# pmh47/dirt

Measured on AMD Instinct MI355X. Metric: forward+backward Mpixels/s at 1024x1024x4ch, 10k-tri mesh, higher is better.
Workload: dtype f32 (f64 edge functions); 1 GPU; K3: rand_mesh F=10000 at 1024x1024x4, 1 scene(s) per GPU, forward+backward; scenes_per_gpu=1, parallelism=batch-sharded x1, no collective, launch=eager (Python wrapper + C ABI per step)

## Files before the change

### dirt_amd/csrc/dirt_forward.hip

```cpp
#include <type_traits>
#include "dirt_device.h"
#include "dirt_launch.h"
#include "dirt_raster_common.h"
#include "../../include/dirt_hip.h"

namespace dirt {

#ifdef DIRT_TRACE
__device__ long long* g_trace_fwd_setup = nullptr;
__device__ long long* g_trace_fwd_raster = nullptr;
extern "C" void dirt_debug_set_trace_forward(void* ps, void* pr)
{
    long long* q = reinterpret_cast<long long*>(ps);
    (void)hipMemcpyToSymbol(HIP_SYMBOL(g_trace_fwd_setup), &q, sizeof(q));
    q = reinterpret_cast<long long*>(pr);
    (void)hipMemcpyToSymbol(HIP_SYMBOL(g_trace_fwd_raster), &q, sizeof(q));
}
#define FMARK() do { if (tr_n < 12) { long long t_; asm volatile("s_memtime %0\n\ts_waitcnt lgkmcnt(0)" : "=s"(t_) :: "memory"); tr_t[tr_n++] = t_; } } while (0)
#define FTRACE_DECL() long long tr_t[12]; int tr_n = 0; const long long tr_wall0 = wall_clock64()
#else
#define FMARK() do {} while (0)
#define FTRACE_DECL() do {} while (0)
#endif

namespace {

constexpr int MAX_FACE_BINS = 16;

__device__ __forceinline__ void glds16(const void* base, uint32_t voff, uint32_t lds_addr)
{
    unsigned keep;
    asm volatile("s_mov_b32 %0, m0\n\ts_mov_b32 m0, %3\n\ts_nop 0\n\tglobal_load_lds_dwordx4 %1, %2\n\ts_mov_b32 m0, %0"
                 : "=&s"(keep) : "v"(voff), "s"(base), "s"(lds_addr) : "memory");
}

#define DIRT_LDS __attribute__((address_space(3)))

constexpr int WAIT_VMCNT_0 = 0x0F70;

template <class T>
__device__ __forceinline__ uint32_t lds_address(T* p)
{
    return (uint32_t)(uintptr_t)(__attribute__((address_space(3))) void*)p;
}

}

constexpr int STHREADS = 256;
template <int CK>
__global__ __launch_bounds__(STHREADS) void setup_kernel_v2(const float* __restrict__ a_vertices, const int32_t* __restrict__ a_faces,
                                                            const float* __restrict__ a_vertex_colors, int a_shared_faces, int a_V, int a_F,
                                                            GeomParams g_in)
{
    GeomParams g = g_in;
    g.vertices = a_vertices; g.faces = a_faces; g.vertex_colors = a_vertex_colors; g.shared_faces = a_shared_faces; g.V = a_V; g.F = a_F;
    __shared__ __align__(16) unsigned long long s_mask[MAX_BINS_MASKED + 2];
    __shared__ __align__(16) FaceRec s_recs[64];
    __shared__ __align__(16) TileRec s_lrecs[64];
    __shared__ __align__(16) float4 s_crecs[CK ? 3 * 64 : 1];
    __shared__ FaceBox s_box[64];
    __shared__ uint8_t s_ok_edges[64], s_ok_box[64];
    const int ib = blockIdx.y, chunk = blockIdx.x, tid = threadIdx.x, lane = tid & 63;
    const int role = __builtin_amdgcn_readfirstlane(tid >> 6);
    FTRACE_DECL();
    FMARK();
    const int nbins = g.grid.bins_x * g.grid.bins_y, big = g.grid.big;
    BinCell* __restrict__ row = g.cells + ((size_t)ib * g.nchunk + chunk) * (size_t)g.grid.cell_chunk_stride;
    if (g.F == 0 || g.V <= 0) {
        for (int i = tid; i <= big; i += STHREADS) if (i < nbins || i == big) row[i] = BinCell{0u, 0u};
        return;
    }
    const int f0 = chunk * 64;
    const int nf = min(64, g.F - f0);
    const size_t n0 = (size_t)ib * g.F + f0;
    const int f = f0 + lane;
    const bool have = lane < nf;
    const int fs = have ? f : 0;
    const float* __restrict__ verts = g.vertices + (size_t)ib * g.V * 4;
    const float* __restrict__ cols = CK ? g.vertex_colors + (size_t)ib * g.V * CK : nullptr;
    auto fetch = [&](int vid) {
        if (role != 3) return *reinterpret_cast<const float4*>(verts + (size_t)vid * 4);
        if constexpr (CK == 0) return make_float4(0.f, 0.f, 0.f, 0.f);
        else {
            const float* __restrict__ cp = cols + (size_t)vid * CK;
            if constexpr (CK == 4) return *reinterpret_cast<const float4*>(cp);
            else if constexpr (CK == 3) { const Float3 q = *reinterpret_cast<const Float3*>(cp); return make_float4(q.x, q.y, q.z, 0.f); }
            else return make_float4(cp[0], 0.f, 0.f, 0.f);
        }
    };
    int32_t idx[3] = {0, 0, 0};
    float4 vv[3];
    const bool fetches = role != 2 && (role != 3 || CK != 0);
    if (fetches) {
        const int32_t* __restrict__ fp = g.faces + (g.shared_faces ? (size_t)fs : (size_t)ib * g.F + fs) * 3;
        idx[0] = fp[0]; idx[1] = fp[1]; idx[2] = fp[2];
#pragma unroll
        for (int k = 0; k < 3; ++k) vv[k] = fetch(min(3 * fs + k, g.V - 1));
    } else if (role == 2) {
        for (int i = lane; i < nbins; i += 64) s_mask[i] = 0ull;
        if (lane == 0) s_mask[big] = 0ull;
    }
    FMARK();
    if (fetches) {
        const bool identity = 3 * fs + 2 < g.V && idx[0] == 3 * fs && idx[1] == 3 * fs + 1 && idx[2] == 3 * fs + 2;
        if (__builtin_amdgcn_ballot_w64(have && !identity) != 0ull) {
#pragma unroll
            for (int k = 0; k < 3; ++k) {
                const int ci = identity ? 3 * fs + k : ((uint32_t)idx[k] < (uint32_t)g.V ? idx[k] : 0);
                vv[k] = fetch(ci);
            }
        }
    }
    FMARK();
    bool ok_mine = false;
    FaceBox box;
    box.i_min = 0; box.i_max = -1; box.r_min = 0; box.r_max = -1;
    if (role == 0) {
        FaceRec rec;
        ok_mine = have && setup_face_edges(vv, idx, g.V, g.H, g.W, rec);
        if (ok_mine) s_recs[lane] = rec;
        else s_recs[lane].flags = 0;
        s_ok_edges[lane] = ok_mine ? 1 : 0;
    } else if (role == 1) {
        ok_mine = have && setup_face_box(vv, g.H, g.W, box);
        s_box[lane] = box;
        s_ok_box[lane] = ok_mine ? 1 : 0;
    } else if (role == 3) {
        if constexpr (CK != 0) { s_crecs[3 * lane] = vv[0]; s_crecs[3 * lane + 1] = vv[1]; s_crecs[3 * lane + 2] = vv[2]; }
    }
    FMARK();
    __syncthreads();
    if (role == 1) {
        if (ok_mine && s_ok_edges[lane]) {
            const unsigned long long bit = 1ull << lane;
            const int bx0 = box.i_min >> g.grid.shift, bx1 = box.i_max >> g.grid.shift;
            const int by0 = box.r_min >> g.grid.shift, by1 = box.r_max >> g.grid.shift;
            if ((bx1 - bx0 + 1) * (by1 - by0 + 1) <= MAX_FACE_BINS) {
                for (int by = by0; by <= by1; ++by)
                    for (int bx = bx0; bx <= bx1; ++bx) atomicOr(&s_mask[by * g.grid.bins_x + bx], bit);
            } else {
                atomicOr(&s_mask[big], bit);
            }
            if (!g.v2_only) {
                BinEntry e;
                e.box = box; e.face = f; e.pad = 0;
                g.entries[((size_t)ib * g.nchunk + chunk) * (5 * (size_t)g.chunk_faces) + lane] = e;
            }
        }
    } else if (role == 2) {
        if (have && s_ok_edges[lane] && s_ok_box[lane]) {
            TileRec lr;
            make_local_rec(s_recs[lane], f, s_box[lane], g.H, (float)g.W, (float)g.H, &lr);
            s_lrecs[lane] = lr;
        }
    } else if (role == 0) {
        const uint4* __restrict__ src = reinterpret_cast<const uint4*>(&s_recs[0]);
        uint4* __restrict__ dst = reinterpret_cast<uint4*>(g.recs + n0);
        for (int i = lane; i < 8 * nf; i += 64) dst[i] = src[i];
    } else {
        if constexpr (CK != 0) {
            const uint4* __restrict__ src = reinterpret_cast<const uint4*>(&s_crecs[0]);
            uint4* __restrict__ dst = reinterpret_cast<uint4*>(g.crecs + 3 * n0);
            for (int i = lane; i < 3 * nf; i += 64) dst[i] = src[i];
        }
    }
    __syncthreads();
    FMARK();
    {
        const uint4* __restrict__ src = reinterpret_cast<const uint4*>(&s_lrecs[0]);
        uint4* __restrict__ dst = reinterpret_cast<uint4*>(g.lrecs + n0);
        for (int i = tid; i < 5 * nf; i += STHREADS) dst[i] = src[i];
    }
    for (int i = 2 * tid; i < nbins; i += 2 * STHREADS) {
        if (i + 1 < nbins) {
            const ulonglong2 m = *reinterpret_cast<const ulonglong2*>(&s_mask[i]);
            *reinterpret_cast<ulonglong2*>(&row[i]) = m;
        } else {
            const unsigned long long m = s_mask[i];
            row[i] = BinCell{(uint32_t)m, (uint32_t)(m >> 32)};
        }
    }
    if (tid == STHREADS - 1) {
        const unsigned long long m = s_mask[big];
        row[big] = BinCell{(uint32_t)m, (uint32_t)(m >> 32)};
    }
    FMARK();
#ifdef DIRT_TRACE
    if (tid == 0 && g_trace_fwd_setup) {
        long long* o = g_trace_fwd_setup + ((size_t)blockIdx.y * gridDim.x + blockIdx.x) * 16;
        for (int i = 0; i < 12; ++i) o[i] = i < tr_n ? tr_t[i] : 0;
        o[12] = tr_wall0; o[13] = (long long)wall_clock64() - tr_wall0;
    }
#endif
}

hipError_t launch_geometry_v2(const GeomParams& g, hipStream_t stream)
{
    const dim3 grid((unsigned)g.nchunk, (unsigned)g.B);
    const int ck = g.crecs ? g.C : 0;
    if (ck == 4) hipLaunchKernelGGL(setup_kernel_v2<4>, grid, dim3(STHREADS), 0, stream, g.vertices, g.faces, g.vertex_colors, g.shared_faces, g.V, g.F, g);
    else if (ck == 3) hipLaunchKernelGGL(setup_kernel_v2<3>, grid, dim3(STHREADS), 0, stream, g.vertices, g.faces, g.vertex_colors, g.shared_faces, g.V, g.F, g);
    else if (ck == 1) hipLaunchKernelGGL(setup_kernel_v2<1>, grid, dim3(STHREADS), 0, stream, g.vertices, g.faces, g.vertex_colors, g.shared_faces, g.V, g.F, g);
    else hipLaunchKernelGGL(setup_kernel_v2<0>, grid, dim3(STHREADS), 0, stream, g.vertices, g.faces, g.vertex_colors, g.shared_faces, g.V, g.F, g);
    return hipGetLastError();
}

namespace {

#ifndef DIRT_V2_CAP
#define DIRT_V2_CAP 96
#endif
constexpr int V2_CAP = DIRT_V2_CAP;

template <bool COLOURS>
struct alignas(16) ShadeSlot {
    double coef[9];
    double inv_det;
    uint32_t flags;
    int32_t vid[3];
    float4 col[COLOURS ? 3 : 0];
};
static_assert(sizeof(ShadeSlot<true>) == 144 && sizeof(ShadeSlot<false>) == 96, "16-byte pieces: 6 of the record, 3 colours");

}

#ifndef DIRT_V2_WAVES
#define DIRT_V2_WAVES 6
#endif
template <int MODE, int CSPEC, int WAVES = 4>
__global__ __launch_bounds__(64 * WAVES, WAVES == 8 ? 8 : DIRT_V2_WAVES) void raster_kernel_v2(
    const BinCell* __restrict__ a_cells, int a_nchunk, int a_tiles_x, int a_tiles_y, uint32_t a_tiles_x_magic, int a_shift, int a_bins_x,
    int a_big, int a_chunk_stride, RasterParams p_in)
{
    RasterParams p = p_in;
    p.cells = a_cells; p.nchunk = a_nchunk; p.tiles_x = a_tiles_x; p.tiles_y = a_tiles_y; p.tiles_x_magic = a_tiles_x_magic;
    p.grid.shift = a_shift; p.grid.bins_x = a_bins_x; p.grid.big = a_big; p.grid.cell_chunk_stride = a_chunk_stride;
    constexpr int NB = 2, NBY = WAVES == 8 ? 1 : 2, TILE = 32, PPL = NB * NBY, THREADS = 64 * WAVES, RH = 8 * NBY;
    constexpr bool COLOURS = MODE == 0;
    constexpr int SPARTS = COLOURS ? 9 : 6;
    using Slot = ShadeSlot<COLOURS>;
    __shared__ __align__(16) TileRec s_rec[V2_CAP];
    __shared__ __align__(16) Slot s_shade[V2_CAP];
    __shared__ int32_t s_face[V2_CAP];
    __shared__ uint32_t s_count;
    FTRACE_DECL();
    FMARK();
#ifdef DIRT_TRACE
    int tr_cand = 0;
#endif
    const int tid = threadIdx.x;
    const int lane = tid & 63;
    const int wave = __builtin_amdgcn_readfirstlane(tid >> 6);
    const int ib = blockIdx.y;
    const int tile = xcd_tile(blockIdx.x, p.tiles_x * p.tiles_y);
    int tile_col, tile_row;
    tile_xy(tile, p.tiles_x, p.tiles_x_magic, tile_col, tile_row);
    const int tx0 = tile_col * TILE, tr0 = tile_row * TILE;
    constexpr int C = CSPEC;

    const FaceRec* __restrict__ recs = p.recs + (size_t)ib * p.F;
    const TileRec* __restrict__ lrecs = p.lrecs + (size_t)ib * p.F;
    const float4* __restrict__ crecs = COLOURS ? p.crecs + (size_t)ib * p.F * 3 : nullptr;
    const int bin = (tr0 >> p.grid.shift) * p.grid.bins_x + (tx0 >> p.grid.shift);
    const BinCell* __restrict__ cells = p.cells + (size_t)ib * p.nchunk * (size_t)p.grid.cell_chunk_stride;
    unsigned long long m_bin = 0ull, m_big = 0ull;
    if (tid < p.nchunk) {
        const BinCell* __restrict__ rowc = cells + (size_t)tid * p.grid.cell_chunk_stride;
        const BinCell a = rowc[bin], b = rowc[p.grid.big];
        m_bin = ((unsigned long long)a.count << 32) | a.start;
        m_big = ((unsigned long long)b.count << 32) | b.start;
    }

    const int wx = wave & 1, wy = wave >> 1;
    const int x0 = tx0 + wx * 16 + (lane & 7);
    const int r0 = tr0 + wy * RH + (lane >> 3);
    double px[NB], py[NBY];
#pragma unroll
    for (int k = 0; k < NB; ++k) px[k] = (double)(x0 + 8 * k) + 0.5;
#pragma unroll
    for (int k = 0; k < NBY; ++k) py[k] = (double)(p.H - 1 - (r0 + 8 * k)) + 0.5;
    unsigned long long best[PPL];
    int cbest[PPL];
#pragma unroll
    for (int k = 0; k < PPL; ++k) { best[k] = (unsigned long long)Z24_CLEAR << 32; cbest[k] = V2_CAP; }
    bool lds_records = true;

    const uint32_t lds_rec = (uint32_t)__builtin_amdgcn_readfirstlane((int)lds_address(&s_rec[0]));
    const uint32_t lds_shade = (uint32_t)__builtin_amdgcn_readfirstlane((int)lds_address(&s_shade[0]));

    FMARK();
    for (int round = 0;; ++round) {
        if (tid == 0) s_count = 0;
        __syncthreads();
        FMARK();
        if (64 * wave < p.nchunk) {
            const uint32_t cnt = (uint32_t)__popcll(m_bin) + (uint32_t)__popcll(m_big);
            uint32_t incl = cnt;
            incl += (uint32_t)__builtin_amdgcn_update_dpp(0, (int)incl, 0x111 , 0xF, 0xF, false);
            incl += (uint32_t)__builtin_amdgcn_update_dpp(0, (int)incl, 0x112 , 0xF, 0xF, false);
            incl += (uint32_t)__builtin_amdgcn_update_dpp(0, (int)incl, 0x114 , 0xF, 0xF, false);
            incl += (uint32_t)__builtin_amdgcn_update_dpp(0, (int)incl, 0x118 , 0xF, 0xF, false);
            incl += (uint32_t)__builtin_amdgcn_update_dpp(0, (int)incl, 0x142 , 0xA, 0xF, false);
            incl += (uint32_t)__builtin_amdgcn_update_dpp(0, (int)incl, 0x143 , 0xC, 0xF, false);
            const uint32_t total = (uint32_t)__builtin_amdgcn_readlane((int)incl, 63);
            uint32_t base = 0;
            if (total != 0u) {
                if (lane == 0) base = atomicAdd(&s_count, total);
                base = (uint32_t)__builtin_amdgcn_readfirstlane((int)base);
            }
            uint32_t slot = base + incl - cnt;
            const int face0 = tid * 64;
            while (m_bin != 0ull && slot < (uint32_t)V2_CAP) {
                s_face[slot++] = face0 + (__ffsll((long long)m_bin) - 1);
                m_bin &= m_bin - 1ull;
            }
            while (m_big != 0ull && slot < (uint32_t)V2_CAP) {
                s_face[slot++] = face0 + (__ffsll((long long)m_big) - 1);
                m_big &= m_big - 1ull;
            }
        }
        FMARK();
        __syncthreads();
        FMARK();
        const int n = (int)min(s_count, (uint32_t)V2_CAP);
        if (round != 0) lds_records = false;

        int tid_o = tid;
        asm volatile("" : "+v"(tid_o));
#pragma unroll
        for (int k = 0; k < (5 * V2_CAP + THREADS - 1) / THREADS; ++k) {
            const int idx = tid_o + THREADS * k;
            if (idx < 5 * n) {
                const int slot = idx / 5, part = idx - 5 * slot;
                glds16(lrecs, (uint32_t)s_face[slot] * (uint32_t)sizeof(TileRec) + 16u * (uint32_t)part, lds_rec + 1024u * (uint32_t)(wave + WAVES * k));
            }
        }
        asm volatile("s_waitcnt vmcnt(0)" ::: "memory");
        FMARK();
        __syncthreads();
        FMARK();
        if (round == 0) {
#pragma unroll
            for (int k = 0; k < (SPARTS * V2_CAP + THREADS - 1) / THREADS; ++k) {
                const int idx = tid_o + THREADS * k;
                if (idx < SPARTS * n) {
                    const int slot = idx / SPARTS, part = idx - SPARTS * slot;
                    const uint32_t face = (uint32_t)s_face[slot];
                    const uint32_t dst = lds_shade + 1024u * (uint32_t)(wave + WAVES * k);
                    if (part < 6) glds16(recs, face * (uint32_t)sizeof(FaceRec) + 16u * (uint32_t)part, dst);
                    if (COLOURS && part >= 6) glds16(crecs, face * 48u + 16u * (uint32_t)(part - 6), dst);
                }
            }
        }

        for (int cb = 0; cb < n; cb += 64) {
            const int idx = cb + lane;
            uint32_t mym4 = 0;
            if (idx < n) {
                const FaceBox box = s_rec[idx].box;
                const int rx0 = tx0 + 16 * wx, ry0 = tr0 + RH * wy;
                const int bx0 = max(box.i_min - rx0, 0) >> 3, bx1 = min(box.i_max - rx0, 15) >> 3;
                const int by0 = max(box.r_min - ry0, 0) >> 3, by1 = min(box.r_max - ry0, RH - 1) >> 3;
                if (box.i_max >= rx0 && box.i_min <= rx0 + 15 && box.r_max >= ry0 && box.r_min <= ry0 + RH - 1) {
                    const uint32_t rowbits = (bx0 == 0 ? 1u : 0u) | (bx1 == 1 ? 2u : 0u);
                    mym4 = (by0 == 0 ? rowbits : 0u) | (NBY == 2 && by1 == 1 ? rowbits << 2 : 0u);
                    mym4 = cull_blocks<NB, NBY>(s_rec[idx], mym4, (float)(rx0 - (int)box.i_min), (float)((int)box.r_min - ry0));
                }
            }
            unsigned long long m = __builtin_amdgcn_ballot_w64(mym4 != 0);
            auto visit = [&](const TileRec& t, int k) {
                const uint32_t m4 = (uint32_t)__builtin_amdgcn_readlane((int)mym4, k);
                float dxl[NB], dyl[NBY];
#pragma unroll
                for (int q = 0; q < NB; ++q) dxl[q] = (float)(x0 + 8 * q - (int)t.box.i_min);
#pragma unroll
                for (int q = 0; q < NBY; ++q) dyl[q] = (float)((int)t.box.r_min - (r0 + 8 * q));
                raster_candidate<NB, NBY>(t, recs, round == 0 ? cb + k : V2_CAP, m4, dxl, dyl, px, py, best, cbest);
#ifdef DIRT_TRACE
                ++tr_cand;
#endif
            };
            while (m) {
                const int k = __ffsll((long long)m) - 1;
                m &= m - 1;
                const TileRec t = s_rec[cb + k];
                visit(t, k);
            }
        }
        FMARK();
        asm volatile("s_waitcnt vmcnt(0)" ::: "memory");
        const bool more = (m_bin | m_big) != 0ull;
        if (!__syncthreads_or(more)) break;
    }
    FMARK();

    int32_t fbest[PPL];
#pragma unroll
    for (int k = 0; k < PPL; ++k) fbest[k] = (uint32_t)(best[k] >> 32) != Z24_CLEAR ? (int32_t)(uint32_t)best[k] : -1;

    const float* __restrict__ cols = COLOURS ? p.vertex_colors + (size_t)ib * p.V * C : nullptr;
    int xs0 = x0, rs0 = r0;
    asm volatile("" : "+v"(xs0), "+v"(rs0));
    const size_t row_base = ((size_t)ib * p.H + tr0) * (size_t)p.W;
    auto pixel_rel = [&](int k, bool& inside) {
        const int x = xs0 + 8 * (k % NB), r = rs0 + 8 * (k / NB);
        inside = x < p.W && r < p.H;
        return (uint32_t)((min(r, p.H - 1) - tr0) * p.W + min(x, p.W - 1));
    };
    const float* __restrict__ bg_base = MODE == 0 ? p.background + row_base * C : nullptr;
    float* __restrict__ out_base = MODE == 0 ? p.pixels + row_base * C : nullptr;
    int32_t* __restrict__ vis_base = p.vis ? p.vis + row_base : nullptr;
    float2* __restrict__ sa_base = p.state_a ? p.state_a + row_base : nullptr;
    float2* __restrict__ sb_base = p.state_a ? p.state_b + row_base : nullptr;
    float4 bgv[PPL];
#pragma unroll
    for (int k = 0; k < PPL; ++k) {
        bool inside;
        const uint32_t rel = pixel_rel(k, inside);
        bgv[k] = make_float4(0.f, 0.f, 0.f, 0.f);
        if (MODE == 0 && inside && fbest[k] < 0) {
            const uint32_t off = rel * (uint32_t)(C * sizeof(float));
            if (CSPEC == 4) bgv[k] = ld_off<float4>(bg_base, off);
            else if (CSPEC == 3) bgv[k] = make_float4(ld_off<float>(bg_base, off), ld_off<float>(bg_base, off + 4u), ld_off<float>(bg_base, off + 8u), 0.f);
            else bgv[k] = make_float4(ld_off<float>(bg_base, off), 0.f, 0.f, 0.f);
        }
    }
    auto shade = [&](auto mem_tag) {
    constexpr bool MEM = decltype(mem_tag)::value;
#pragma unroll
    for (int k = 0; k < PPL; ++k) {
        const int32_t f = fbest[k];
        const bool has = f >= 0;
        const bool from_lds = has && lds_records && cbest[k] < V2_CAP;
        const int ci = from_lds ? cbest[k] : 0;
        const DIRT_LDS Slot* sl = (const DIRT_LDS Slot*)&s_shade[ci];
        double cf[9];
#pragma unroll
        for (int i = 0; i < 9; ++i) cf[i] = sl->coef[i];
        uint32_t flags = sl->flags;
        double inv_det = sl->inv_det;
        const bool from_mem = has && !from_lds;
        if constexpr (MEM) {
            if (from_mem) {
                const FaceRec* __restrict__ rec = recs + f;
#pragma unroll
                for (int i = 0; i < 9; ++i) cf[i] = rec->coef[i];
                flags = rec->flags; inv_det = rec->inv_det;
            }
        }
        double Fk[3];
        edge_eval(cf, (double)(xs0 + 8 * (k % NB)) + 0.5, (double)(p.H - 1 - (rs0 + 8 * (k / NB))) + 0.5, Fk);
        float b[3], cw;
        bary_eval(Fk, flags, inv_det, b, cw);
        const float b0 = b[0], b1 = b[1], b2 = b[2];
        float u[3][4] = {};
        if constexpr (COLOURS) {
            const DIRT_LDS float* cl = (const DIRT_LDS float*)&s_shade[ci].col[0];
#pragma unroll
            for (int i = 0; i < 12; ++i) u[i / 4][i % 4] = cl[i];
            if constexpr (MEM) {
                if (from_mem) {
                    const FaceRec* __restrict__ rec = recs + f;
#pragma unroll
                    for (int v = 0; v < 3; ++v) {
                        const float* __restrict__ cv = cols + (size_t)rec->vid[v] * C;
#pragma unroll
                        for (int c = 0; c < C; ++c) u[v][c] = cv[c];
                    }
                }
            }
        }
        if (MODE == 0 && k == 0) __builtin_amdgcn_s_waitcnt(WAIT_VMCNT_0);
        float4 o = bgv[k];
        if (MODE == 0 && has) {
            o.x = fmaf(b2, u[2][0], fmaf(b1, u[1][0], b0 * u[0][0]));
            if (CSPEC >= 3) { o.y = fmaf(b2, u[2][1], fmaf(b1, u[1][1], b0 * u[0][1])); o.z = fmaf(b2, u[2][2], fmaf(b1, u[1][2], b0 * u[0][2])); }
            if (CSPEC == 4) o.w = fmaf(b2, u[2][3], fmaf(b1, u[1][3], b0 * u[0][3]));
        }
        bool inside;
        const uint32_t rel = pixel_rel(k, inside);
        if (!inside) continue;
        if (p.vis) st_off<int32_t>(vis_base, rel * 4u, f);
        if (p.state_a) store_state(sa_base, sb_base, rel * 8u, has, b0, b1, b2, cw, f);
        if (MODE != 0) continue;
        const uint32_t off = rel * (uint32_t)(C * sizeof(float));
        if (CSPEC == 4) st_off<float4>(out_base, off, o);
        else if (CSPEC == 3) { st_off<float>(out_base, off, o.x); st_off<float>(out_base, off + 4u, o.y); st_off<float>(out_base, off + 8u, o.z); }
        else st_off<float>(out_base, off, o.x);
    }
    };
    bool some_from_mem = false;
#pragma unroll
    for (int k = 0; k < PPL; ++k) some_from_mem |= fbest[k] >= 0 && !(lds_records && cbest[k] < V2_CAP);
    if (__builtin_amdgcn_ballot_w64(some_from_mem) != 0ull) shade(std::true_type());
    else shade(std::false_type());
    if ((p.zero_b_bytes | p.zero_c_bytes) != 0) {
        const unsigned gwg = blockIdx.y * gridDim.x + blockIdx.x;
        if (p.zero_b_bytes) zero_share<THREADS>(p.zero_b, p.zero_b_bytes, p.zero_b_per, gwg, tid);
        if (p.zero_c_bytes) zero_share<THREADS>(p.zero_c, p.zero_c_bytes, p.zero_c_per, gwg, tid);
    }
    FMARK();
#ifdef DIRT_TRACE
    if (lane == 0 && g_trace_fwd_raster) {
        long long* o = g_trace_fwd_raster + (((size_t)blockIdx.y * gridDim.x + blockIdx.x) * WAVES + wave) * 16;
        for (int i = 0; i < 12; ++i) o[i] = i < tr_n ? tr_t[i] : 0;
        o[12] = tr_wall0; o[13] = (long long)wall_clock64() - tr_wall0; o[14] = blockIdx.x; o[15] = tr_cand;
    }
#endif
}

int raster_tile_choice(int H, int W, int B, unsigned flags)
{
    const long long tiles32 = (long long)((W + 31) / 32) * ((H + 31) / 32) * B;
    int tile = tiles32 >= 512 ? 32 : 16;
    if (flags & DIRT_FLAG_TILES_SMALL) tile = 16;
    if (flags & DIRT_FLAG_TILES_LARGE) tile = 32;
    return tile;
}

bool raster_v2_applies(const RasterParams& p, int B, bool visibility_only)
{
    if (!p.masked || p.lrecs == nullptr) return false;
    if (raster_tile_choice(p.H, p.W, B, p.flags) != 32) return false;
    if (visibility_only) return true;
    return (p.C == 1 || p.C == 3 || p.C == 4) && p.crecs != nullptr;
}

hipError_t launch_raster_v2(const RasterParams& p_in, int B, bool visibility_only, hipStream_t stream)
{
    RasterParams p = p_in;
    set_tile_grid(p, 32, 32);
    const dim3 grid((unsigned)(p.tiles_x * p.tiles_y), (unsigned)B);
    {
        const size_t nwg = (size_t)grid.x * grid.y;
        p.zero_b_per = (unsigned)((p.zero_b_bytes / 16 + nwg - 1) / nwg);
        p.zero_c_per = (unsigned)((p.zero_c_bytes / 16 + nwg - 1) / nwg);
    }
    const bool pinned8 = (p.flags & (DIRT_FLAG_TILES_LARGE | DIRT_FLAG_TILES_SMALL)) == (DIRT_FLAG_TILES_LARGE | DIRT_FLAG_TILES_SMALL);
    const bool w8 = !visibility_only && (pinned8 || ((size_t)grid.x * grid.y <= 2048 && !(p.flags & DIRT_FLAG_TILES_LARGE)));
#define V2_ARGS p.cells, p.nchunk, p.tiles_x, p.tiles_y, p.tiles_x_magic, p.grid.shift, p.grid.bins_x, p.grid.big, p.grid.cell_chunk_stride, p
    if (visibility_only) hipLaunchKernelGGL((raster_kernel_v2<1, 4>), grid, dim3(RTHREADS), 0, stream, V2_ARGS);
    else if (w8 && p.C == 4) hipLaunchKernelGGL((raster_kernel_v2<0, 4, 8>), grid, dim3(512), 0, stream, V2_ARGS);
    else if (w8 && p.C == 3) hipLaunchKernelGGL((raster_kernel_v2<0, 3, 8>), grid, dim3(512), 0, stream, V2_ARGS);
    else if (w8) hipLaunchKernelGGL((raster_kernel_v2<0, 1, 8>), grid, dim3(512), 0, stream, V2_ARGS);
    else if (p.C == 4) hipLaunchKernelGGL((raster_kernel_v2<0, 4>), grid, dim3(RTHREADS), 0, stream, V2_ARGS);
    else if (p.C == 3) hipLaunchKernelGGL((raster_kernel_v2<0, 3>), grid, dim3(RTHREADS), 0, stream, V2_ARGS);
    else hipLaunchKernelGGL((raster_kernel_v2<0, 1>), grid, dim3(RTHREADS), 0, stream, V2_ARGS);
#undef V2_ARGS
    return hipGetLastError();
}

}
```

### dirt_amd/csrc/dirt_raster_common.h

```cpp
#pragma once
#include "dirt_device.h"
#include "dirt_launch.h"

namespace dirt {

constexpr int RTHREADS = 256;
constexpr int LIST_CAP = 1024;
constexpr int SHADE_CAP = 96;
struct alignas(8) ShadeRec {
    double coef[9];
    double inv_det;
    uint32_t flags;
    int32_t vid[3];
    double pad;
};
static_assert(sizeof(ShadeRec) == 104, "ShadeRec is 26 dwords");

struct alignas(16) TileRec {
    float a[3], b[3], c[3];
    float bound;
    FaceBox box;
    double zp[3];
    uint32_t flags;
    int32_t face;
};
static_assert(sizeof(TileRec) == 80, "TileRec is 80 bytes");

__device__ __forceinline__ void make_tile_rec(const FaceRec& rec, int face, double ox, double oy, float wf, float hf, TileRec* out)
{
    const uint32_t flags = rec.flags;
    float bound = 0.f;
#pragma unroll
    for (int k = 0; k < 3; ++k) {
        const double a = rec.coef[3 * k], b = rec.coef[3 * k + 1], c = rec.coef[3 * k + 2];
        const double cl = fma(a, ox, fma(b, oy, c));
        const float sg = (flags & (1u << k)) ? -1.f : 1.f;
        const float a32 = (float)a, b32 = (float)b, c32 = (float)cl, cg = (float)c;
        const float mg = fabsf(a32) * wf + fabsf(b32) * hf + fabsf(cg);
        const float bnd = (0x1p-22f * (32.f * fabsf(a32) + 32.f * fabsf(b32) + fabsf(c32)) + 0x1p-49f * mg) * 1.0001f;
        bound = (bnd > bound || bnd != bnd) ? bnd : bound;
        out->a[k] = sg * a32; out->b[k] = sg * b32; out->c[k] = sg * c32;
    }
    out->bound = bound; out->box.i_min = 0; out->box.i_max = 0; out->box.r_min = 0; out->box.r_max = 0;
    out->zp[0] = rec.zp[0]; out->zp[1] = rec.zp[1]; out->zp[2] = rec.zp[2];
    out->flags = flags; out->face = face;
}

__device__ __forceinline__ void make_local_rec(const FaceRec& rec, int face, const FaceBox& box, int H, float wf, float hf, TileRec* out)
{
    const uint32_t flags = rec.flags;
    const double ox = (double)box.i_min + 0.5, oy = (double)(H - 1 - box.r_min) + 0.5;
    const float D = (float)(max(box.i_max - box.i_min, box.r_max - box.r_min) + 8);
    float bound = 0.f;
#pragma unroll
    for (int k = 0; k < 3; ++k) {
        const double a = rec.coef[3 * k], b = rec.coef[3 * k + 1], c = rec.coef[3 * k + 2];
        const double cl = fma(a, ox, fma(b, oy, c));
        const float sg = (flags & (1u << k)) ? -1.f : 1.f;
        const float a32 = (float)a, b32 = (float)b, c32 = (float)cl, cg = (float)c;
        const float mg = fabsf(a32) * wf + fabsf(b32) * hf + fabsf(cg);
        const float bnd = (0x1p-22f * (D * fabsf(a32) + D * fabsf(b32) + fabsf(c32)) + 0x1p-49f * mg) * 1.0001f;
        bound = (bnd > bound || bnd != bnd) ? bnd : bound;
        out->a[k] = sg * a32; out->b[k] = sg * b32; out->c[k] = sg * c32;
    }
    out->bound = bound; out->box = box;
    out->zp[0] = rec.zp[0]; out->zp[1] = rec.zp[1]; out->zp[2] = rec.zp[2];
    out->flags = flags; out->face = face;
}

template <int NB, int NBY = NB>
__device__ __forceinline__ uint32_t cull_blocks(const TileRec& t, uint32_t m4, float dx_lo0, float dy_hi0)
{
    const float nb = -t.bound;
#pragma unroll
    for (int by = 0; by < NBY; ++by) {
        const float dy_hi = dy_hi0 - 8.f * (float)by, dy_lo = dy_hi - 7.f;
#pragma unroll
        for (int bx = 0; bx < NB; ++bx) {
            const float dx_lo = dx_lo0 + 8.f * (float)bx, dx_hi = dx_lo + 7.f;
            bool out = false;
#pragma unroll
            for (int k = 0; k < 3; ++k) {
                const float e = fmaf(t.a[k], t.a[k] > 0.f ? dx_hi : dx_lo, fmaf(t.b[k], t.b[k] > 0.f ? dy_hi : dy_lo, t.c[k]));
                out |= e < nb;
            }
            if (out) m4 &= ~(1u << (NB * by + bx));
        }
    }
    return m4;
}

static __device__ __noinline__ bool covered_exact(const FaceRec* __restrict__ rec, double px, double py)
{
    const uint32_t flags = rec->flags;
    const double F0 = fma(rec->coef[0], px, fma(rec->coef[1], py, rec->coef[2]));
    const double F1 = fma(rec->coef[3], px, fma(rec->coef[4], py, rec->coef[5]));
    const double F2 = fma(rec->coef[6], px, fma(rec->coef[7], py, rec->coef[8]));
    return ((F0 >= 0.0) != ((flags & 1u) != 0)) && ((F1 >= 0.0) != ((flags & 2u) != 0)) && ((F2 >= 0.0) != ((flags & 4u) != 0));
}

template <int NB, int NBY = NB>
__device__ __forceinline__ void raster_candidate(const TileRec& t, const FaceRec* __restrict__ recs, int ci, uint32_t m4, const float* dx,
                                                 const float* dy, const double* px, const double* py, unsigned long long* best,
                                                 int* cbest)
{
#pragma unroll
    for (int by = 0; by < NBY; ++by) {
        if (!((m4 >> (NB * by)) & ((1u << NB) - 1u))) continue;
        float trow[3];
        trow[0] = fmaf(t.b[0], dy[by], t.c[0]);
        trow[1] = fmaf(t.b[1], dy[by], t.c[1]);
        trow[2] = fmaf(t.b[2], dy[by], t.c[2]);
        const double qrow = fma(t.zp[1], py[by], t.zp[2]);
#pragma unroll
        for (int bx = 0; bx < NB; ++bx) {
            const int k = NB * by + bx;
            if (!((m4 >> k) & 1u)) continue;
            const float E0 = fmaf(t.a[0], dx[bx], trow[0]);
            const float E1 = fmaf(t.a[1], dx[bx], trow[1]);
            const float E2 = fmaf(t.a[2], dx[bx], trow[2]);
            const float m = fminf(fminf(E0, E1), E2);
            unsigned long long cov_m = __builtin_amdgcn_ballot_w64(m > t.bound);
            const unsigned long long unsure_m = __builtin_amdgcn_ballot_w64(!(m < -t.bound)) & ~cov_m;
            if (__builtin_expect(unsure_m != 0ull, 0)) {
                bool c = false;
                if (__builtin_amdgcn_inverse_ballot_w64(unsure_m)) c = covered_exact(recs + t.face, px[bx], py[by]);
                cov_m |= __builtin_amdgcn_ballot_w64(c);
            }
            if (cov_m == 0ull) continue;
            const double q = fma(t.zp[0], px[bx], qrow);
            const uint32_t z24 = (uint32_t)__double_as_longlong(q + 4503599627370496.0);
            const unsigned long long in_range_m = __builtin_amdgcn_ballot_w64((unsigned long long)__double_as_longlong(q) <= 0x416FFFFFE0000000ull);
            const unsigned long long key = ((unsigned long long)z24 << 32) | (unsigned long long)(uint32_t)t.face;
            const unsigned long long wins_m = cov_m & in_range_m & __builtin_amdgcn_ballot_w64(key < best[k]);
            const bool wins = __builtin_amdgcn_inverse_ballot_w64(wins_m);
            best[k] = wins ? key : best[k];
            cbest[k] = wins ? ci : cbest[k];
        }
    }
}

__device__ __forceinline__ void raster_candidate_pair(const TileRec& t0, const TileRec& t1, const FaceRec* __restrict__ recs, int ci0, int ci1,
                                                      float dx, float dy, double px, double py, unsigned long long& best, int& cbest)
{
    const float E00 = fmaf(t0.a[0], dx, fmaf(t0.b[0], dy, t0.c[0])), E10 = fmaf(t1.a[0], dx, fmaf(t1.b[0], dy, t1.c[0]));
    const float E01 = fmaf(t0.a[1], dx, fmaf(t0.b[1], dy, t0.c[1])), E11 = fmaf(t1.a[1], dx, fmaf(t1.b[1], dy, t1.c[1]));
    const float E02 = fmaf(t0.a[2], dx, fmaf(t0.b[2], dy, t0.c[2])), E12 = fmaf(t1.a[2], dx, fmaf(t1.b[2], dy, t1.c[2]));
    const float m0 = fminf(fminf(E00, E01), E02), m1 = fminf(fminf(E10, E11), E12);
    unsigned long long cov0 = __builtin_amdgcn_ballot_w64(m0 > t0.bound), cov1 = __builtin_amdgcn_ballot_w64(m1 > t1.bound);
    const unsigned long long uns0 = __builtin_amdgcn_ballot_w64(!(m0 < -t0.bound)) & ~cov0, uns1 = __builtin_amdgcn_ballot_w64(!(m1 < -t1.bound)) & ~cov1;
    if (__builtin_expect((uns0 | uns1) != 0ull, 0)) {
        bool c0 = false, c1 = false;
        if (__builtin_amdgcn_inverse_ballot_w64(uns0)) c0 = covered_exact(recs + t0.face, px, py);
        if (__builtin_amdgcn_inverse_ballot_w64(uns1)) c1 = covered_exact(recs + t1.face, px, py);
        cov0 |= __builtin_amdgcn_ballot_w64(c0); cov1 |= __builtin_amdgcn_ballot_w64(c1);
    }
    if ((cov0 | cov1) == 0ull) return;
    const double q0 = fma(t0.zp[0], px, fma(t0.zp[1], py, t0.zp[2])), q1 = fma(t1.zp[0], px, fma(t1.zp[1], py, t1.zp[2]));
    const uint32_t z0 = (uint32_t)__double_as_longlong(q0 + 4503599627370496.0), z1 = (uint32_t)__double_as_longlong(q1 + 4503599627370496.0);
    const unsigned long long in0 = __builtin_amdgcn_ballot_w64((unsigned long long)__double_as_longlong(q0) <= 0x416FFFFFE0000000ull);
    const unsigned long long in1 = __builtin_amdgcn_ballot_w64((unsigned long long)__double_as_longlong(q1) <= 0x416FFFFFE0000000ull);
    const unsigned long long key0 = ((unsigned long long)z0 << 32) | (unsigned long long)(uint32_t)t0.face;
    const unsigned long long key1 = ((unsigned long long)z1 << 32) | (unsigned long long)(uint32_t)t1.face;
    const bool w0 = __builtin_amdgcn_inverse_ballot_w64(cov0 & in0 & __builtin_amdgcn_ballot_w64(key0 < best));
    const unsigned long long b1 = w0 ? key0 : best;
    const int c1i = w0 ? ci0 : cbest;
    const bool w1 = __builtin_amdgcn_inverse_ballot_w64(cov1 & in1 & __builtin_amdgcn_ballot_w64(key1 < b1));
    best = w1 ? key1 : b1;
    cbest = w1 ? ci1 : c1i;
}

__device__ __forceinline__ void store_state(float2* plane_a, float2* plane_b, uint32_t off, bool has, float b0, float b1, float b2, float clip_w, int32_t face)
{
    *reinterpret_cast<float2*>(reinterpret_cast<char*>(plane_a) + off) = make_float2(has ? clip_w : INFINITY, __int_as_float(face));
    *reinterpret_cast<float2*>(reinterpret_cast<char*>(plane_b) + off) = has ? encode_bary(b0, b1, b2) : make_float2(-1.f, -1.f);
}
__device__ __forceinline__ void store_state(const RasterParams& p, size_t pix, bool has, float b0, float b1, float b2, float clip_w, int32_t face)
{
    store_state(p.state_a + pix, p.state_b + pix, 0u, has, b0, b1, b2, clip_w, face);
}

template <int NTHREADS = RTHREADS>
__device__ __forceinline__ void zero_share(void* buf, size_t bytes, unsigned per, unsigned gwg, int tid)
{
    const size_t units = bytes / 16;
    const size_t i0 = (size_t)gwg * per;
    uint4* q = reinterpret_cast<uint4*>(buf);
    for (unsigned i = (unsigned)tid; i < per; i += NTHREADS)
        if (i0 + i < units) q[i0 + i] = make_uint4(0u, 0u, 0u, 0u);
    if (gwg == 0 && (size_t)tid < (bytes % 16) / 4) reinterpret_cast<uint32_t*>(buf)[units * 4 + tid] = 0u;
}

}
```

Measured before the change: 24380 Mpixels/s.

## Vectorize tile record LDS fetch and prioritize busy waves in raster loop

Tile records are now read from LDS with explicit volatile 128-bit loads, and the face and flags fields swap places to match that layout. The per-block offsets are computed incrementally from a single conversion, and the slot index uses an OR mask instead of a select. Waves with many candidate faces raise their scheduling priority through s_setprio, a compiler assume is added on the block mask, and the mask bit clear uses s_bitset0. The aim is to cut LDS instruction count and per-candidate scalar overhead and to even out load imbalance between waves, at the cost of the volatile loads blocking compiler reordering.

```diff
diff --git a/dirt_amd/csrc/dirt_forward.hip b/dirt_amd/csrc/dirt_forward.hip
--- a/dirt_amd/csrc/dirt_forward.hip
+++ b/dirt_amd/csrc/dirt_forward.hip
@@ -42,6 +42,31 @@
 __device__ __forceinline__ uint32_t lds_address(T* p)
 {
     return (uint32_t)(uintptr_t)(__attribute__((address_space(3))) void*)p;
+}
+
+typedef float f32x4 __attribute__((ext_vector_type(4)));
+typedef double f64x2 __attribute__((ext_vector_type(2)));
+typedef uint32_t u32x4 __attribute__((ext_vector_type(4)));
+static_assert(offsetof(TileRec, bound) == 36 && offsetof(TileRec, box) == 40 && offsetof(TileRec, zp) == 48 && offsetof(TileRec, face) == 72,
+              "fetch_rec reads TileRec by offsets");
+
+__device__ __forceinline__ TileRec fetch_rec(const TileRec* rec)
+{
+    const volatile DIRT_LDS char* q = (const volatile DIRT_LDS char*)rec;
+    const f32x4 p0 = *(const volatile DIRT_LDS f32x4*)(q + 0);
+    const f32x4 p1 = *(const volatile DIRT_LDS f32x4*)(q + 16);
+    const u32x4 p2 = *(const volatile DIRT_LDS u32x4*)(q + 32);
+    const f64x2 p3 = *(const volatile DIRT_LDS f64x2*)(q + 48);
+    const u32x4 p4 = *(const volatile DIRT_LDS u32x4*)(q + 64);
+    TileRec t;
+    t.a[0] = p0.x; t.a[1] = p0.y; t.a[2] = p0.z; t.b[0] = p0.w;
+    t.b[1] = p1.x; t.b[2] = p1.y; t.c[0] = p1.z; t.c[1] = p1.w;
+    t.c[2] = __uint_as_float(p2.x); t.bound = __uint_as_float(p2.y);
+    t.box.i_min = (int16_t)(p2.z & 0xFFFFu); t.box.i_max = (int16_t)(p2.z >> 16);
+    t.box.r_min = (int16_t)(p2.w & 0xFFFFu); t.box.r_max = (int16_t)(p2.w >> 16);
+    t.zp[0] = p3.x; t.zp[1] = p3.y; t.zp[2] = __longlong_as_double((long long)(((unsigned long long)p4.y << 32) | p4.x));
+    t.face = (int32_t)p4.z; t.flags = p4.w;
+    return t;
 }
 
 }
@@ -353,6 +378,8 @@
             }
         }
 
+        const int slot_gone = round == 0 ? 0 : 128;
+        static_assert(V2_CAP <= 128, "slot_gone must put a slot past V2_CAP");
         for (int cb = 0; cb < n; cb += 64) {
             const int idx = cb + lane;
             uint32_t mym4 = 0;
@@ -370,22 +397,31 @@
             unsigned long long m = __builtin_amdgcn_ballot_w64(mym4 != 0);
             auto visit = [&](const TileRec& t, int k) {
                 const uint32_t m4 = (uint32_t)__builtin_amdgcn_readlane((int)mym4, k);
+                if (NBY == 1) __builtin_assume((m4 & 3u) != 0u);
                 float dxl[NB], dyl[NBY];
-#pragma unroll
-                for (int q = 0; q < NB; ++q) dxl[q] = (float)(x0 + 8 * q - (int)t.box.i_min);
-#pragma unroll
-                for (int q = 0; q < NBY; ++q) dyl[q] = (float)((int)t.box.r_min - (r0 + 8 * q));
-                raster_candidate<NB, NBY>(t, recs, round == 0 ? cb + k : V2_CAP, m4, dxl, dyl, px, py, best, cbest);
+                dxl[0] = (float)(x0 - (int)t.box.i_min);
+                dyl[0] = (float)((int)t.box.r_min - r0);
+#pragma unroll
+                for (int q = 1; q < NB; ++q) dxl[q] = dxl[0] + 8.f * (float)q;
+#pragma unroll
+                for (int q = 1; q < NBY; ++q) dyl[q] = dyl[0] - 8.f * (float)q;
+                raster_candidate<NB, NBY>(t, recs, (cb + k) | slot_gone, m4, dxl, dyl, px, py, best, cbest);
 #ifdef DIRT_TRACE
                 ++tr_cand;
 #endif
             };
+            if constexpr (WAVES == 8) {
+                const int nv = __popcll(m);
+                if (nv >= 14) __builtin_amdgcn_s_setprio(3);
+                else if (nv >= 10) __builtin_amdgcn_s_setprio(2);
+                else if (nv >= 7) __builtin_amdgcn_s_setprio(1);
+            }
             while (m) {
                 const int k = __ffsll((long long)m) - 1;
-                m &= m - 1;
-                const TileRec t = s_rec[cb + k];
-                visit(t, k);
-            }
+                asm("s_bitset0_b64 %0, %1" : "+s"(m) : "s"(k));
+                visit(fetch_rec(&s_rec[cb + k]), k);
+            }
+            if constexpr (WAVES == 8) __builtin_amdgcn_s_setprio(0);
         }
         FMARK();
         asm volatile("s_waitcnt vmcnt(0)" ::: "memory");
diff --git a/dirt_amd/csrc/dirt_raster_common.h b/dirt_amd/csrc/dirt_raster_common.h
--- a/dirt_amd/csrc/dirt_raster_common.h
+++ b/dirt_amd/csrc/dirt_raster_common.h
@@ -21,8 +21,8 @@
     float bound;
     FaceBox box;
     double zp[3];
+    int32_t face;
     uint32_t flags;
-    int32_t face;
 };
 static_assert(sizeof(TileRec) == 80, "TileRec is 80 bytes");
 
```

Measured after the change: 25270 Mpixels/s (median of 6 runs). +3.7%, better.
